# johannesulf/TabCorr

Measured on AMD Instinct MI355X. Metric: predict_calls_per_sec, higher is better.
Workload: dtype f64; 1 GPU; BASELINE configs[1]: Zheng07 predict(), synthetic auto table 50 mass bins x {cen,sat} (G=100, P=5050), 19 rp bins, n_gauss_prim=10, batch of 10000 draws per GPU per step, draws and results resident in HBM; n_tables=1, gather=none, gather_payload=ngal + xi (160 B per draw), gather_every_steps=32, lanes=4, rccl_ranks=0

## Files before the change

### include/tabcorr_amd_testing.h

```cpp
#ifndef TABCORR_AMD_TESTING_H
#define TABCORR_AMD_TESTING_H

#include "tabcorr_amd.h"

#ifdef __cplusplus
extern "C" {
#endif

int tc_debug_fastmath(int kind, int64_t n, const double* x, double* y);

int tc_debug_central_series(int n_gauss, double log_min, double log_max, double dist_index,
                            int64_t n, const double* log_m_min, const double* sigma,
                            double* series, double* nodes, int32_t* terms);

int tc_debug_satellite_series(int n_gauss, double log_min, double log_max, double dist_index,
                              int64_t n, const double* log_m0, const double* log_m1,
                              const double* alpha, double* series, double* nodes,
                              int32_t* terms);

int tc_plan_debug(int mode, int n_bins, const uint8_t* is_central, int n_chunks,
                  int64_t* n_entries, int32_t* entry_pair, int32_t* entry_chunk,
                  int32_t* entry_class);

int tc_debug_quad_schedule(int n_bins, int n_central, int by_type, int n_tiles, int n_rtiles,
                           int n_tables, int separate, int max_waves, int min_units,
                           int order ,
                           int* n_waves, int* n_runs, int* n_slabs, int64_t* units_min,
                           int64_t* units_max);
int tc_debug_triangle_parts(int n_rb, int n_parts, int32_t* rb0, int32_t* cb0, int32_t* count);
int tc_debug_node_groups(int n_bins, int n_central, const double* log_min,
                         const double* log_max, int32_t* begin, int32_t* member,
                         int* n_groups, int* n_central_groups);
int tc_debug_quad_emulate(int n_bins, int n_r, const double* tpcf_matrix,
                          const uint8_t* is_central, int by_type, int separate,
                          const double* densities, int64_t ldb, int64_t n_draws,
                          int max_waves, int min_units, int order, double* out);

int tc_debug_trace(tc_table* table, uint64_t* out, int64_t capacity, int64_t* n_blocks);
int tc_debug_wave_trace(tc_table* table, uint64_t* out, int64_t capacity,
                        int64_t* n_waves);
int tc_debug_resident_ticks(tc_table* table, uint64_t* out, int64_t capacity, int64_t* n_blocks);
int tc_debug_ensemble_stamps(tc_table* table, uint64_t* out);
#ifdef __cplusplus
}
// ... 4 lines not shown
```

### tabcorr_amd/_lib.py

```python

import ctypes
import os

import numpy as np

HERE = os.path.dirname(os.path.abspath(__file__))
LIBRARY = os.path.join(HERE, 'libtabcorr_hip.so')

TC_OK = 0
TC_ERR_INVALID = 1
TC_ERR_HIP = 2
TC_ERR_UNSUPPORTED = 3
TC_ERR_RCCL = 4

MODE = {'auto': 0, 'cross': 1}
DTYPE_F64 = 0
DTYPE_F32 = 1

FLAG_SEPARATE_GAL_TYPE = 1
FLAG_MODULATE_WITH_CENOCC = 2
FLAG_ASSEMBIAS = 4
FLAG_LEAUTHAUD11 = 16

UNIQUE_ID_BYTES = 128
# ... 18 lines not shown
    'tc_memcpy_h2d': [ctypes.c_void_p, ctypes.c_void_p, ctypes.c_size_t],
    'tc_memcpy_d2h': [ctypes.c_void_p, ctypes.c_void_p, ctypes.c_size_t],
    'tc_host_alloc': [c_void_pp, ctypes.c_size_t],
    'tc_host_free': [ctypes.c_void_p],
    'tc_host_register': [ctypes.c_void_p, ctypes.c_size_t],
    'tc_host_unregister': [ctypes.c_void_p],
    'tc_host_is_pinned': [ctypes.c_void_p, ctypes.c_size_t, c_int_p],
    'tc_gauss_legendre': [ctypes.c_int, c_double_p, c_double_p],
    'tc_debug_fastmath': [ctypes.c_int, ctypes.c_int64, c_double_p,
                          c_double_p],
    'tc_pair_indices': [ctypes.c_int, c_int32_p, c_int32_p, c_int32_p],
    'tc_spline_interpolation_matrix': [ctypes.c_int, c_double_p, c_double_p],
    'tc_plan_debug': [ctypes.c_int, ctypes.c_int, c_uint8_p, ctypes.c_int,
                      c_int64_p, c_int32_p, c_int32_p, c_int32_p],
    'tc_debug_triangle_parts': [ctypes.c_int, ctypes.c_int, c_int_p, c_int_p, c_int_p],
    'tc_debug_central_series': [ctypes.c_int, ctypes.c_double, ctypes.c_double, ctypes.c_double,
                                ctypes.c_int64, c_double_p, c_double_p, c_double_p, c_double_p,
                                c_int32_p],
    'tc_debug_satellite_series': [ctypes.c_int, ctypes.c_double, ctypes.c_double,
                                  ctypes.c_double, ctypes.c_int64, c_double_p, c_double_p,
                                  c_double_p, c_double_p, c_double_p, c_int32_p],
    'tc_debug_node_groups': [ctypes.c_int, ctypes.c_int, c_double_p, c_double_p,
                             c_int32_p, c_int32_p, c_int_p, c_int_p],
    'tc_debug_quad_schedule': [ctypes.c_int] * 10 + [c_int_p, c_int_p, c_int_p,
                                                     c_int64_p, c_int64_p],
    'tc_debug_quad_emulate': [ctypes.c_int, ctypes.c_int, c_double_p, c_uint8_p,
                              ctypes.c_int, ctypes.c_int, c_double_p,
                              ctypes.c_int64, ctypes.c_int64, ctypes.c_int,
                              ctypes.c_int, ctypes.c_int, c_double_p],
    'tc_table_create': [
# ... 210 lines not shown
```

### tabcorr_amd/csrc/hostmath.cpp

```cpp
#include "hostmath.h"
#include "fastmath.h"
#include "series.h"

#include <algorithm>
#include <atomic>
#include <cmath>
#include <cstring>
#include <map>
#include <numeric>
#include <tuple>
#include <thread>

namespace tc {

void gauss_legendre(int n, std::vector<double>& x, std::vector<double>& w) {
  x.assign(n, 0.0);
  w.assign(n, 0.0);
  const long double pi = 3.141592653589793238462643383279502884L;
  for (int i = 0; i < (n + 1) / 2; ++i) {
    long double z = cosl(pi * (i + 0.75L) / (n + 0.5L));
    long double dp = 1.0L;
    for (int iter = 0; iter < 100; ++iter) {
      long double p0 = 1.0L, p1 = z;
      for (int k = 2; k <= n; ++k) {
// ... 704 lines not shown
}

void triangle_parts(int n_rb, int n_parts, int32_t* rb0, int32_t* cb0, int32_t* count) {
  const int64_t n_units = (int64_t)n_rb * (n_rb + 1) / 2;
  for (int part = 0; part < n_parts; ++part) {
    const int64_t begin = n_units * part / n_parts, end = n_units * (part + 1) / n_parts;
    int64_t rb = (int64_t)((std::sqrt(8.0 * (double)begin + 1.0) - 1.0) / 2.0);
    while ((rb + 1) * (rb + 2) / 2 <= begin) ++rb;
    while (rb * (rb + 1) / 2 > begin) --rb;
    rb0[part] = (int32_t)rb;
    cb0[part] = (int32_t)(begin - rb * (rb + 1) / 2);
    count[part] = (int32_t)(end - begin);
  }
}

QuadTiling quad_tiling(int n_r) {
  QuadTiling tiling;
  tiling.n_rtiles = (n_r + 19) / 20;
  tiling.r_per_tile = (n_r + tiling.n_rtiles - 1) / tiling.n_rtiles;
  tiling.n_u = (tiling.r_per_tile + 3) / 4;
  return tiling;
}

void fill_quad_table(const QuadLayout& layout, const std::vector<int32_t>& perm, int n_r,
                     int64_t n_pairs, const void* matrix, bool matrix_is_f32,
                     const QuadTiling& tiling, std::vector<double>& out) {
  const int up = (tiling.n_u + 1) / 2;
  const size_t per_unit = (size_t)up * 128;
  out.assign((size_t)tiling.n_rtiles * layout.n_units * per_unit, 0.0);
  auto source = [&](int r, int64_t column) {
// ... 478 lines not shown
```

### tabcorr_amd/csrc/hostmath.h

```cpp
#pragma once

#include <cstdint>
#include <string>
#include <vector>

namespace tc {

void gauss_legendre(int n, std::vector<double>& x, std::vector<double>& w);

inline int64_t packed_index(int64_t i, int64_t j) {
  return i >= j ? i * (i + 1) / 2 + j : j * (j + 1) / 2 + i;
}

bool spline_interpolation_matrix(int n, const double* xp, std::vector<double>& a);

struct Segment {
  int32_t component;
  int32_t rectangular;
  int32_t i_lo, i_hi;
  int32_t j_lo, j_hi;
  int64_t q_begin;
  int64_t n_real;
};

// ... 114 lines not shown
  int32_t pad;
};
struct QuadMergePlan {
  int waves_per_block = 0;
  int n_blocks = 0;
  int lds_slots = 0;
  std::vector<int32_t> block_begin;
  std::vector<QuadMerge> merges;
};
void merge_quad_schedule(const QuadLayout& layout, int n_rtiles, bool separate,
                         int waves_per_block, int max_slots, QuadSchedule& schedule,
                         QuadMergePlan& plan);

void triangle_parts(int n_rb, int n_parts, int32_t* rb0, int32_t* cb0, int32_t* count);

struct QuadTiling {
  int n_rtiles = 1;
  int r_per_tile = 0;
  int n_u = 0;
};
QuadTiling quad_tiling(int n_r);

void fill_quad_table(const QuadLayout& layout, const std::vector<int32_t>& perm, int n_r,
                     int64_t n_pairs, const void* matrix, bool matrix_is_f32,
                     const QuadTiling& tiling, std::vector<double>& out);

QuadTiling quad_tiling_f32(int n_r);
void fill_quad_table_f32(const QuadLayout& layout, const std::vector<int32_t>& perm, int n_r,
                         int64_t n_pairs, const void* matrix, bool matrix_is_f32,
                         const QuadTiling& tiling, std::vector<float>& out);
// ... 47 lines not shown
```

### tabcorr_amd/csrc/internal.h

```cpp
#pragma once

#include <hip/hip_runtime.h>
#include <hip/hip_ext.h>

#include <algorithm>
#include <chrono>
#include <cmath>
#include <cstdarg>
#include <cstdio>
#include <cstdlib>
#include <cstring>
#include <map>
#include <memory>
#include <string>
#include <utility>
#include <vector>

#include "../../include/tabcorr_amd.h"
#include "../../include/tabcorr_amd_testing.h"
#include "fastmath.h"
#include "hostmath.h"
#include "kernel_args.h"

namespace tc {
// ... 217 lines not shown
  int occ_splits = 0;
  int occ_per_cu = 4;
  int n_groups = 0, n_waves = 0, lds_min = 0, min_chunk_entries = 32;
  int k_splits = 0;
  int trace = 0;
  int autotune_after = 0;
  int sync_chunks = 0;
  int sync_form = 32;
  int sync_stagger = 10;
  int sync_direct_out = 2;
  int async_direct_in = 1;
  int async_direct_out = 2;
  int series = -1;
  int cross_defer = 1;
  int fused_defer = 2;
  int fused_sat_cap = 6;
  int cross_wide_min_draws = 4096;
  int cross_target = 160;
  int resident_aperture = 1;
  int cross_min_draws = 192;
  int fused = 1;
  int fused_min_draws = 0;
  int fused_max_draws = 30720;
  int fused_waves = 0;
  int fused_draws = 0;
  int fused_spread = 1, fused_spread_min = 8192, fused_spread_rounds = 1;
  int prio_fused = 1, prio_fused_occ = 2, prio_fused_out = 3;
  int deterministic = 0;
  int skip_occ = 0, skip_finalize = 0;
  void load() {
// ... 63 lines not shown
  int n_r = 0;
  int64_t n_pairs = 0;
  int compute_dtype = TC_DTYPE_F64;
  bool legacy = false;
  tc::Plan plan;
  int rt = 0;
  int n_rtiles = 0;
  hipStream_t stream = nullptr;
  hipEvent_t ev_begin = nullptr, ev_end = nullptr;

  std::vector<double> n_h, log_min, log_max, percentile, dist_index;

  void* d_table = nullptr;
  size_t table_bytes = 0;
  void* d_n_h = nullptr;
  void* d_percentile = nullptr;
  void* d_perm = nullptr;
  tc::NodeGroups node_groups;
  void* d_group_begin = nullptr;
  void* d_group_member = nullptr;
  void* d_group_n_h = nullptr;
  void* d_group_percentile = nullptr;
  bool grouped = false;
  void* d_math_table = nullptr;
  void* d_pos_ij = nullptr;
  void* d_pos_off = nullptr;
  std::vector<double> cross_host;
  tc::host::CrossFused cross_fused, cross_fused_wide;
  int sync_cross_target = 0;
  std::vector<hipEvent_t> chunk_events;
// ... 225 lines not shown
```

### tabcorr_amd/csrc/kernel_args.h

```cpp
#pragma once

#include <cstdint>

#include "hostmath.h"

namespace tc {

constexpr int kLanes = 64;
constexpr unsigned kFlagSeparate = 1u;
constexpr unsigned kFlagModulate = 2u;
constexpr unsigned kFlagAssembias = 4u;
constexpr int kOccWaves = 4;
constexpr int kF32Block = 8;
constexpr int kF64Block = 8;
constexpr int kF32Tile = 32;
constexpr int kFinalizeRows = 32;
constexpr int kMaxInterpDim = 8;
constexpr int kMaxInterpAxis = 32;

struct GroupArgs {
  const int32_t* begin;
  const int32_t* member;
  const double* log_m;
  const double* m;
// ... 218 lines not shown
struct FusedArgs {
  const double* theta;
  int n_theta;
  int n_bins;
  int n_central;
  int n_gauss;
  int dens_rows;
  int part_rb0[kFusedMaxParts];
  int part_cb0[kFusedMaxParts];
  int part_count[kFusedMaxParts];
  int part_triangular[kFusedMaxParts];
  int part_n_cb[kFusedMaxParts];
  int part_i_row0[kFusedMaxParts];
  int part_j_row0[kFusedMaxParts];
  int part_unit_base[kFusedMaxParts];
  int separate;
  int n_r;
  int priority;
  int64_t n_draws;
  const double* log_m;
  const double* m;
  const double* weight;
  const double* n_h;
  const double* percentile;
  double split;
  const double* math_table;
  const void* table;
  uint32_t table_bytes;
  double* ngal;
  double* xi;
// ... 114 lines not shown
```

### tabcorr_amd/csrc/kernels.hip.h

```cpp
#pragma once

#include <hip/hip_runtime.h>

#include <cstdint>
#include <utility>

#include "fastmath.h"
#include "hostmath.h"
#include "kernel_args.h"
#include "series.h"

#ifdef TC_DEVELOPER_KNOBS
#define TC_TRACE(pointer) ((pointer) != nullptr)
#else
#define TC_TRACE(pointer) false
#endif

namespace tc {

static_assert(sizeof(QuadRun) == 32 && sizeof(QuadCompArgs) == 32, "read as 8 x int32");

typedef const __attribute__((address_space(4))) double* sc_f64;
typedef const __attribute__((address_space(4))) float* sc_f32;
typedef const __attribute__((address_space(4))) int32_t* sc_i32;
// ... 1892 lines not shown
      mma(t1, b1, false);
      __builtin_amdgcn_sched_barrier(0);
    } else {
      t0 = t1;
      b0 = b1;
    }
#pragma unroll
    for (int u = 0; u < UU; ++u)
#pragma unroll
      for (int v = 0; v < 4; ++v) {
        F[u][0] = fma(D[u][0][v], e[v].x, F[u][0]);
        F[u][1] = fma(D[u][1][v], e[v].y, F[u][1]);
      }
    ++rb;
    cb = 0;
  }
}

__device__ __forceinline__ int wave_prefix_sum(int value) {
  auto shifted = [](int x, auto control, auto rows) {
    return __builtin_amdgcn_update_dpp(0, x, decltype(control)::value, decltype(rows)::value, 0xf,
                                       false);
  };
  typedef std::integral_constant<int, 0xf> all_rows;
  value += shifted(value, std::integral_constant<int, 0x111>(), all_rows());
  value += shifted(value, std::integral_constant<int, 0x112>(), all_rows());
  value += shifted(value, std::integral_constant<int, 0x114>(), all_rows());
  value += shifted(value, std::integral_constant<int, 0x118>(), all_rows());
  value += shifted(value, std::integral_constant<int, 0x142>(), std::integral_constant<int, 0xa>());
  value += shifted(value, std::integral_constant<int, 0x143>(), std::integral_constant<int, 0xc>());
// ... 138 lines not shown
      stamps[blockIdx.x * 32 + which] = __builtin_amdgcn_s_memrealtime();
  };
  if (skip & 1)
    for (int idx = threadIdx.x; idx < a.n_bins * DL; idx += blockDim.x) fused_lds[idx] = 1e-3;
#else
  constexpr int skip = 0;
  const int n_bins_occ = a.n_bins;
  auto stamp = [](int) {};
  auto wave_stamp = [](int) {};
#endif
  stamp(0);
  set_priority((a.priority >> 2) & 3);
  const int lane = threadIdx.x & 63;
  const int wave = __builtin_amdgcn_readfirstlane(threadIdx.x >> 6);
  const int n_gauss = NGAUSS > 0 ? NGAUSS : a.n_gauss;
  {
    typedef double __attribute__((ext_vector_type(2))) double2v;
    const int hi = fm::kTableDoubles / 2;
    const double2v* src = (const double2v*)a.math_table;
    double2v* dst = (double2v*)table;
    for (int i = threadIdx.x; i < hi; i += blockDim.x) dst[i] = src[i];
  }
  for (int idx = a.n_bins * DL + threadIdx.x; idx < a.dens_rows * DL; idx += blockDim.x)
    dens[idx] = 0.0;
  __syncthreads();
  stamp(1);

  const int draw = DL != 32 ? lane : (lane & 31);
  const int half = DL != 32 ? 0 : (lane >> 5);
  const bool live = DL != 40 || lane < 40;
  auto dens_at = [&](int row, int d) -> double& {
    return dens[DL == 40 ? dens40(row, d) : row * DL + d];
  };
  const int64_t col = (int64_t)blockIdx.x * DL;
  const int64_t b0 = col + draw;
  const int64_t b = b0 < a.n_draws ? b0 : a.n_draws - 1;
  double norm;
  {
    const double* th = a.theta + b * a.n_theta;
    LeauthaudDraw ld;
    if (LEAUTHAUD) ld = prepare_leauthaud(table, kc, th);
    DrawParams dp = LEAUTHAUD ? prepare_draw(table, kc, 12.0, 1.0, 12.0, 13.0, 1.0, 0.0, 0.0)
                              : draw_params<ASSEMBIAS>(table, kc, th);
    series_setup<MODULATE>(dp, (GROUPED ? a.group.series : a.series) != nullptr && DL != 32,
                           (GROUPED ? a.group.sat_series : a.sat_series) != nullptr && DL != 32);
    sc_f64 log_m = (sc_f64)a.log_m;
    sc_f64 mass = (sc_f64)a.m;
    sc_f64 weight = (sc_f64)a.weight;
    sc_f64 weight_sum = weight + a.n_bins * n_gauss;
    sc_f64 n_h = (sc_f64)a.n_h;
    sc_f64 percentile = (sc_f64)a.percentile;
// ... 160 lines not shown
    stamp(3);
    red[0][wave][lane] = sum_cen;
    red[1][wave][lane] = sum_sat;
    __syncthreads();
    stamp(4);
    double n_cen = 0.0, n_sat = 0.0;
#pragma unroll
    for (int w = 0; w < W; ++w) {
      n_cen += red[0][w][lane];
      n_sat += red[1][w][lane];
    }
    const double total = (skip & 1) ? 1.0 : n_cen + n_sat;
    norm = total * total;
    if (wave == 0 && half == 0 && live && b0 < a.n_draws) {
      if (a.separate) {
        a.ngal[2 * b0] = n_cen;
        a.ngal[2 * b0 + 1] = n_sat;
      } else {
        a.ngal[b0] = total;
      }
    }
  }

  set_priority(a.priority & 3);
  const int c = lane & 15, kq = lane >> 4;
  double F[UP][2][2];
  constexpr int UA = DL == 40 ? (U > 3 ? 3 : U) : 1, UB = DL == 40 && U > 3 ? U - 3 : 1;
  double F40a[UA][10], F40b[UB][10];
  if (DL == 40) {
    const int part = wave;
    const unsigned off_a = ((lane & 0x30) | ((lane & 3) << 2) | ((lane >> 2) & 3)) * 16;
    const double* dens_b = dens + (a.part_j_row0[part] + (lane >> 4)) * 40 + (lane & 3) * 10;
    const double* dens_e = dens + (a.part_i_row0[part] + (lane >> 4)) * 40 + (lane & 3) * 10;
    const __amdgpu_buffer_rsrc_t rs_t =
// ... 23 lines not shown
    if (U > 3 && !(skip & 2))
      fused_quad_pass40<(U > 3 ? 3 : 0), UB>(rs_t, off_a, unit_bytes, dens_b, dens_e, rb, cb,
                                             count, triangular, n_cb, first_unit, F40b);
  } else {
    const int sub = wave / PARTS, part = wave % PARTS;
    const unsigned off_a = lane * 16;
    const double* dens_b =
        dens + (a.part_j_row0[part] + kq) * DL + sub * kQuadTile + 2 * c;
    const double* dens_e = dens + a.part_i_row0[part] * DL + sub * kQuadTile + 2 * c;
    const __amdgpu_buffer_rsrc_t rs_t =
        __builtin_amdgcn_make_buffer_rsrc((void*)a.table, 0, a.table_bytes, kBufferFlags);
    const int rb = a.part_rb0[part], cb = a.part_cb0[part], count = a.part_count[part];
    const bool triangular = a.part_triangular[part] != 0;
    const int n_cb = a.part_n_cb[part];
    const unsigned unit_base = (unsigned)a.part_unit_base[part];
#pragma unroll
    for (int p = 0; p < UP; ++p) {
      F[p][0][0] = F[p][0][1] = F[p][1][0] = F[p][1][1] = 0.0;
      if (skip & 2) continue;
      if (2 * p + 1 < U)
        fused_quad_pass<2, DL>(rs_t, off_a + p * 1024, UP * 1024, dens_b, dens_e, rb, cb, count,
                               triangular, n_cb, unit_base, F[p]);
      else
        fused_quad_pass<1, DL>(rs_t, off_a + p * 1024, UP * 1024, dens_b, dens_e, rb, cb, count,
                               triangular, n_cb, unit_base, F[p]);
    }
  }
  stamp(5);
  __syncthreads();
  stamp(8);
  if (DL == 40) {
    const int q = lane >> 4;
    auto share = [&](int sub, int g) {
      return sub < UA ? F40a[sub < UA ? sub : 0][g] : F40b[sub >= UA ? sub - UA : 0][g];
    };
    double* out = dens + (wave * (4 * U) + ((lane >> 2) & 3)) * 40 + (lane & 3);
    if (((a.priority >> 11) & 1) && __builtin_amdgcn_ballot_w64(!(norm < 1e280)) == 0) {
      double select[4];
#pragma unroll
      for (int m = 0; m < 4; ++m) select[m] = (lane & 3) == m ? 1.0 : 0.0;
#pragma unroll
      for (int sub = 0; sub < U; ++sub)
#pragma unroll
        for (int t = 0; t < 3; ++t) {
          double sums = 0.0;
// ... 77 lines not shown
    const int rows = a.n_r;
    const double* data = chi2_lds;
    const double* matrix = chi2_lds + rows;
    double part = 0.0;
    for (int i = wave; i < rows; i += W) {
      double inner = 0.0;
      for (int j = 0; j < rows; ++j)
        inner = fma(matrix[i * rows + j], tile[j][lane] - data[j], inner);
      part = fma(tile[i][lane] - data[i], inner, part);
    }
    red[0][wave][lane] = part;
    __syncthreads();
    if (wave == 0 && lane < n_valid) {
      double total = 0.0;
      for (int w = 0; w < W; ++w) total += red[0][w][lane];
      a.chi2[col + lane] = total;
    }
    return;
  }
  for (int idx = threadIdx.x; idx < a.n_r * DL; idx += blockDim.x) {
    const int d = idx / a.n_r, rr = idx % a.n_r;
    if (d < n_valid) a.xi[(col + d) * (int64_t)a.n_r + rr] = tile[rr][d];
  }
  stamp(7);
}

template <int ROW_LANES, typename Coefficient>
__device__ __forceinline__ void cross_deferred_pairs(
    const CrossFusedArgs& a, const double* table, const fm::Consts& kc, const DrawParams& dp,
    const unsigned long long* bitmap, unsigned* list, int wave, int lane, int g_first, int g_last,
    int type, Coefficient&& coefficient, double* res) {
  constexpr int SHARES = 64 / ROW_LANES;
  constexpr int SLOTS = 8 / SHARES;
  const int row = lane % ROW_LANES, share = lane / ROW_LANES;
  const unsigned long long owner = 0x0101010101010101ull << wave;
  double extra[SLOTS];
#pragma unroll
// ... 1787 lines not shown
```

### tabcorr_amd/csrc/launch.hip

```cpp
#include <immintrin.h>

#include <atomic>
#include <mutex>

#include "internal.h"
#include "kernels.hip.h"
#include "series.h"

namespace tc {
namespace host {

int get_quadrature(tc_table* t, int n_gauss, Quadrature** out) {
  auto it = t->quadrature.find(n_gauss);
  if (it != t->quadrature.end()) {
    *out = &it->second;
    return TC_OK;
  }
  std::vector<double> x, w;
  tc::gauss_legendre(n_gauss, x, w);
  const int g = t->n_bins;
  std::vector<double> log_m((size_t)g * n_gauss), m((size_t)g * n_gauss),
      weight((size_t)g * n_gauss + g);
  for (int i = 0; i < g; ++i) {
    const double d_log = t->log_max[i] - t->log_min[i];
// ... 916 lines not shown
  fa.n_theta = n_theta;
  fa.n_bins = t->n_bins;
  fa.n_central = t->plan.n_central;
  fa.n_gauss = n_gauss;
  fa.dens_rows = fused_dens_rows(t, separate);
  fa.separate = separate ? 1 : 0;
  const bool spread = fused_spread_eligible(t, n_draws, n_gauss, flags);
  const bool wide = !spread && fused_wide_tables(t, separate, n_gauss, flags);
  const bool half_tiles = !spread && !wide && fused_half_tiles(t, separate, n_draws, n_gauss, flags);
  const int waves = spread || wide || half_tiles ? 8 : fused_waves(t, separate, flags);
  const int draws = spread ? 40 : wide || half_tiles ? 32 : 64;
  const int n_parts = spread ? 8 : waves * 32 / draws;
  if (!separate) {
    const tc::QuadComp& comp = q_table.layout.comps[0];
    tc::triangle_parts(comp.n_rb, n_parts, fa.part_rb0, fa.part_cb0, fa.part_count);
    for (int part = 0; part < n_parts; ++part) {
      fa.part_triangular[part] = 1;
      fa.part_n_cb[part] = comp.n_cb;
      fa.part_i_row0[part] = comp.i_bin0;
      fa.part_j_row0[part] = comp.j_bin0;
      fa.part_unit_base[part] = (int)comp.unit_base;
    }
  } else {
    const int quarter = n_parts / 4;
    for (int part = 0; part < n_parts; ++part) {
      const int c = part < quarter ? 0 : part < 3 * quarter ? 1 : 2;
      const int first = c == 0 ? 0 : c == 1 ? quarter : 3 * quarter;
      const int pieces = c == 1 ? 2 * quarter : quarter, piece = part - first;
      const tc::QuadComp& comp = q_table.layout.comps[c];
      fa.part_triangular[part] = comp.triangular;
// ... 9 lines not shown
        fa.part_count[part] = count[piece];
      } else {
        const int64_t begin = comp.n_units * piece / pieces;
        const int64_t end = comp.n_units * (piece + 1) / pieces;
        fa.part_rb0[part] = (int)(begin / comp.n_cb);
        fa.part_cb0[part] = (int)(begin % comp.n_cb);
        fa.part_count[part] = (int)(end - begin);
      }
    }
  }
  fa.n_r = t->n_r;
  fa.priority = (t->tuning.prio_fused & 3) | ((t->tuning.prio_fused_occ & 3) << 2) |
                ((t->tuning.prio_fused_out & 3) << 4) |
                ((env_int_early("TC_FUSED_SKIP", 0) & 3) << 8) |
                (q_table.finite ? 1 << 11 : 0);
  fa.n_draws = n_draws;
  fa.n_groups = t->node_groups.n_groups;
  fa.n_central_groups = t->node_groups.n_central_groups;
  fa.group = group_args(t, *q);
  fa.series = (series_mask(t) & 1) ? (const double*)q->series : nullptr;
  fa.series_thr = (const int32_t*)q->series_thr;
  fa.sat_series = (series_mask(t) & 2) ? (const double*)q->sat_series : nullptr;
  fa.sat_series_thr = (const int32_t*)q->sat_series_thr;
  fa.log_m = (const double*)q->log_m;
  fa.m = (const double*)q->m;
  fa.weight = (const double*)q->weight;
  fa.n_h = (const double*)t->d_n_h;
  fa.percentile = (const double*)t->d_percentile;
  fa.split = 0.5;
  fa.math_table = (const double*)t->d_math_table;
// ... 994 lines not shown
```

### tabcorr_amd/csrc/runtime.cpp

```cpp
#include <dlfcn.h>
#include <pthread.h>

#include <atomic>
#include <condition_variable>
#include <mutex>
#include <new>
#include <thread>
#include <vector>

#include "internal.h"
#include "series.h"

namespace tc {
namespace host {

namespace {
thread_local std::string g_last_error;
}

namespace {
struct Roctx {
  int (*push)(const char*) = nullptr;
  int (*pop)() = nullptr;
};
// ... 631 lines not shown
        entry_chunk[e] = c;
        entry_class[e] = chunk.component;
        ++e;
      }
    }
  }
  for (int64_t q = 0; q < plan.n_positions; ++q)
    if (!seen[q]) return fail(TC_ERR_INVALID, "position %lld not covered", (long long)q);
  if (e != plan.n_entries) return fail(TC_ERR_INVALID, "entries missing");
  return TC_OK;
}

int tc_debug_triangle_parts(int n_rb, int n_parts, int32_t* rb0, int32_t* cb0, int32_t* count) {
  TC_CHECK(n_rb >= 1 && n_parts >= 1 && rb0 && cb0 && count, "invalid argument");
  tc::triangle_parts(n_rb, n_parts, rb0, cb0, count);
  return TC_OK;
}

int tc_debug_quad_schedule(int n_bins, int n_central, int by_type, int n_tiles, int n_rtiles,
                           int n_tables, int separate, int max_waves, int min_units, int order,
                           int* n_waves, int* n_runs, int* n_slabs, int64_t* units_min,
                           int64_t* units_max) {
  TC_CHECK(n_bins >= 1 && n_central >= 0 && n_central <= n_bins && n_tiles >= 1 &&
               n_rtiles >= 1 && max_waves >= 1,
           "invalid arguments");
  tc::QuadLayout layout;
  tc::build_quad_layout(n_bins, n_central, by_type != 0, layout);
  tc::QuadSchedule schedule;
  tc::build_quad_schedule(layout, n_tiles, n_rtiles, n_tables, separate != 0, max_waves,
                          min_units, schedule, order);
// ... 91 lines not shown
```

### tabcorr_amd/csrc/table.cpp

```cpp
#include <cmath>

#include "internal.h"

using namespace tc::host;

extern "C" {

int tc_table_create(int mode, int n_bins, int n_r, int64_t n_pairs,
                    const void* tpcf_matrix, int matrix_dtype, const double* n_h,
                    const double* log_min, const double* log_max,
                    const double* percentile, const double* dist_index,
                    const uint8_t* is_central, int compute_dtype, tc_table** out) {
  TC_CHECK(out != nullptr, "table output pointer is NULL");
  *out = nullptr;
  TC_CHECK(mode == TC_MODE_AUTO || mode == TC_MODE_CROSS, "invalid mode %d", mode);
  TC_CHECK(n_bins >= 1 && n_bins < (1 << 20), "invalid number of bins %d", n_bins);
  TC_CHECK(n_r >= 1, "invalid number of correlation function bins %d", n_r);
  const int64_t expect =
      mode == TC_MODE_AUTO ? (int64_t)n_bins * (n_bins + 1) / 2 : n_bins;
  TC_CHECK(n_pairs == expect,
           "tpcf_matrix has %lld columns but %d bins in mode '%s' need %lld",
           (long long)n_pairs, n_bins, mode == TC_MODE_AUTO ? "auto" : "cross",
           (long long)expect);
  TC_CHECK(n_pairs < (1LL << 31), "too many pair columns");
// ... 113 lines not shown
    for (int l = 0; l < t->n_lanes; ++l) t->lanes[l].stream = streams[l];
    if (created != TC_OK) return created;
    for (int l = 0; l < t->n_lanes; ++l)
      TC_HIP(hipEventCreateWithFlags(&t->lanes[l].finished, hipEventDisableTiming));
  }
  t->stream = t->lanes[0].stream;
  TC_HIP(hipEventCreate(&t->ev_begin));
  TC_HIP(hipEventCreate(&t->ev_end));
  int status = compute_dtype == TC_DTYPE_F64 ? upload(tmp64, &t->d_table)
                                             : upload(tmp32, &t->d_table);
  if (status == TC_OK && compute_dtype == TC_DTYPE_F32)
    status = upload(pos_ij, &t->d_pos_ij);
  if (status == TC_OK && compute_dtype == TC_DTYPE_F64)
    status = upload(pos_ij, &t->d_pos_off);
  if (status == TC_OK) status = upload(t->n_h, &t->d_n_h);
  if (status == TC_OK) status = upload(t->percentile, &t->d_percentile);
  if (status == TC_OK) status = upload(t->plan.perm, &t->d_perm);
  tc::find_node_groups(n_bins, t->plan.n_central, t->log_min.data(), t->log_max.data(),
                       t->node_groups);
  t->grouped = t->node_groups.largest > 1;
  if (status == TC_OK) status = upload(t->node_groups.begin, &t->d_group_begin);
  if (status == TC_OK) status = upload(t->node_groups.member, &t->d_group_member);
  {
    std::vector<double> n_h_m, percentile_m;
    for (int32_t g : t->node_groups.member) {
      n_h_m.push_back(t->n_h[g]);
      percentile_m.push_back(t->percentile[g]);
    }
    if (status == TC_OK) status = upload(n_h_m, &t->d_group_n_h);
    if (status == TC_OK) status = upload(percentile_m, &t->d_group_percentile);
// ... 26 lines not shown

int tc_table_destroy(tc_table* t) {
  if (t == nullptr) return TC_OK;
  (void)hipSetDevice(t->device);
  (void)resident_stop(t);
  if (t->resident.stream) (void)hipStreamDestroy(t->resident.stream);
  t->resident.mailbox.release();
  t->resident.ens_mailbox.release();
  t->resident.ens_out.release();
  t->resident.ens_device.release();
  t->resident.ens_aperture.release();
  t->resident.single_aperture.release();
  t->resident.ws.buffer.release();
  for (tc_table::Lane& lane : t->lanes)
    if (lane.stream) (void)hipStreamSynchronize(lane.stream);
  for (void* p : {t->d_table, t->d_n_h, t->d_percentile, t->d_perm, t->d_math_table,
                  t->d_pos_ij, t->d_pos_off, t->d_group_begin, t->d_group_member,
                  t->d_group_n_h, t->d_group_percentile})
    if (p) (void)hipFree(p);
  for (auto& kv : t->quadrature)
    for (void* p : {kv.second.log_m, kv.second.m, kv.second.weight, kv.second.group_log_m,
                    kv.second.group_m, kv.second.group_weight, kv.second.series,
                    kv.second.series_thr, kv.second.group_series, kv.second.group_series_thr,
                    kv.second.sat_series, kv.second.sat_series_thr, kv.second.group_sat_series,
                    kv.second.group_sat_series_thr, kv.second.group_records, kv.second.sat_records, kv.second.cen_records})
      if (p) (void)hipFree(p);
  for (auto& kv : t->chunkings)
    for (void* p : {kv.second->chunks, kv.second->groups})
      if (p) (void)hipFree(p);
  t->quad_by_type.release();
  t->quad_total.release();
// ... 1073 lines not shown
  } else if (key == "resident_aperture") {
    TC_CHECK(value == 0 || value == 1, "resident_aperture must be 0 or 1");
    const int status = resident_stop(t);
    if (status != TC_OK) return status;
    t->tuning.resident_aperture = value;
    t->resident.ens_grid = 0;
    t->resident.single_aperture_decided = false;
  } else if (key == "cross_min_draws") {
    TC_CHECK(value >= 1, "cross_min_draws must be positive");
    t->tuning.cross_min_draws = value;
  } else if (key == "cross_defer") {
    t->tuning.cross_defer = value != 0;
  } else if (key == "fused_defer") {
    TC_CHECK(value >= 0 && value <= 2, "fused_defer must be 0, 1 or 2");
    t->tuning.fused_defer = value;
  } else if (key == "fused_sat_cap") {
    TC_CHECK(value >= 0 && value <= 6, "fused_sat_cap must be in [0, 6]");
    t->tuning.fused_sat_cap = value;
  } else if (key == "cross_wide_min_draws") {
    TC_CHECK(value >= 0, "cross_wide_min_draws must not be negative");
    t->tuning.cross_wide_min_draws = value;
  } else if (key == "cross_target") {
    TC_CHECK(value >= 1 && value <= 4096, "cross_target must be in [1, 4096]");
    t->tuning.cross_target = value;
  } else if (key == "series") {
    TC_CHECK(value >= -1 && value <= 3, "series must be -1 .. 3");
    t->tuning.series = value;
  } else if (key == "grouped") {
    t->grouped = value != 0 && t->node_groups.largest > 1;
  } else if (key == "lanes") {
// ... 215 lines not shown
```

Before: 271.9 million calls/s.

## Skip empty density blocks in fused quad and sort draws by satellite cutoff

Adds a row-set based quadrature pass for the non-separate fused kernel that ballots which 4-bin density blocks are nonzero across the wave and skips MFMA work on dead blocks. To make those blocks dead for whole waves, each block ranks draws by how many satellite block upper mass limits their log_M0 exceeds, using an in-LDS counting sort, and processes draws in that sorted order, scattering ngal, xi and chi2 back to the original indices. Rows are assigned to parts by greedy balancing instead of contiguous triangle ranges. The cost is a per-block histogram/rank prologue over all draws and more irregular control flow in the MFMA loop.

```diff
diff --git a/include/tabcorr_amd_testing.h b/include/tabcorr_amd_testing.h
--- a/include/tabcorr_amd_testing.h
+++ b/include/tabcorr_amd_testing.h
@@ -28,6 +28,8 @@
                            int* n_waves, int* n_runs, int* n_slabs, int64_t* units_min,
                            int64_t* units_max);
 int tc_debug_triangle_parts(int n_rb, int n_parts, int32_t* rb0, int32_t* cb0, int32_t* count);
+
+int tc_debug_triangle_row_parts(int n_rb, int n_parts, uint64_t* rows);
 int tc_debug_node_groups(int n_bins, int n_central, const double* log_min,
                          const double* log_max, int32_t* begin, int32_t* member,
                          int* n_groups, int* n_central_groups);
diff --git a/tabcorr_amd/_lib.py b/tabcorr_amd/_lib.py
--- a/tabcorr_amd/_lib.py
+++ b/tabcorr_amd/_lib.py
@@ -56,6 +56,8 @@
     'tc_plan_debug': [ctypes.c_int, ctypes.c_int, c_uint8_p, ctypes.c_int,
                       c_int64_p, c_int32_p, c_int32_p, c_int32_p],
     'tc_debug_triangle_parts': [ctypes.c_int, ctypes.c_int, c_int_p, c_int_p, c_int_p],
+    'tc_debug_triangle_row_parts': [ctypes.c_int, ctypes.c_int,
+                                    ctypes.POINTER(ctypes.c_uint64)],
     'tc_debug_central_series': [ctypes.c_int, ctypes.c_double, ctypes.c_double, ctypes.c_double,
                                 ctypes.c_int64, c_double_p, c_double_p, c_double_p, c_double_p,
                                 c_int32_p],
diff --git a/tabcorr_amd/csrc/hostmath.cpp b/tabcorr_amd/csrc/hostmath.cpp
--- a/tabcorr_amd/csrc/hostmath.cpp
+++ b/tabcorr_amd/csrc/hostmath.cpp
@@ -742,6 +742,31 @@
   }
 }
 
+void triangle_row_parts(int n_rb, int n_parts, uint64_t* rows) {
+  std::vector<int64_t> units(n_parts, 0);
+  for (int part = 0; part < n_parts; ++part) rows[part] = 0;
+  int above = -1;
+  for (int rb = n_rb - 1; rb >= 0; --rb) {
+    int best = -1;
+    for (int part = 0; part < n_parts; ++part)
+      if ((part != above || n_parts == 1) && (best < 0 || units[part] < units[best])) best = part;
+    units[best] += rb + 1;
+    rows[best] |= (uint64_t)1 << rb;
+    above = best;
+  }
+}
+
+void satellite_block_tops(int n_bins, int n_central, const double* log_max,
+                          std::vector<double>& tops) {
+  tops.clear();
+  for (int first = (n_central + 3) / 4 * 4; first < n_bins; first += 4) {
+    double top = log_max[first];
+    for (int g = first; g < n_bins && g < first + 4; ++g) top = std::max(top, log_max[g]);
+    if (top == top) tops.push_back(top);
+  }
+  std::sort(tops.begin(), tops.end());
+}
+
 QuadTiling quad_tiling(int n_r) {
   QuadTiling tiling;
   tiling.n_rtiles = (n_r + 19) / 20;
diff --git a/tabcorr_amd/csrc/hostmath.h b/tabcorr_amd/csrc/hostmath.h
--- a/tabcorr_amd/csrc/hostmath.h
+++ b/tabcorr_amd/csrc/hostmath.h
@@ -152,6 +152,11 @@
 
 void triangle_parts(int n_rb, int n_parts, int32_t* rb0, int32_t* cb0, int32_t* count);
 
+void triangle_row_parts(int n_rb, int n_parts, uint64_t* rows);
+
+void satellite_block_tops(int n_bins, int n_central, const double* log_max,
+                          std::vector<double>& tops);
+
 struct QuadTiling {
   int n_rtiles = 1;
   int r_per_tile = 0;
diff --git a/tabcorr_amd/csrc/internal.h b/tabcorr_amd/csrc/internal.h
--- a/tabcorr_amd/csrc/internal.h
+++ b/tabcorr_amd/csrc/internal.h
@@ -255,6 +255,7 @@
   int series = -1;
   int cross_defer = 1;
   int fused_defer = 2;
+  int fused_skip = 1;
   int fused_sat_cap = 6;
   int cross_wide_min_draws = 4096;
   int cross_target = 160;
@@ -348,6 +349,8 @@
   void* d_table = nullptr;
   size_t table_bytes = 0;
   void* d_n_h = nullptr;
+  std::vector<double> block_tops;
+  void* d_block_tops = nullptr;
   void* d_percentile = nullptr;
   void* d_perm = nullptr;
   tc::NodeGroups node_groups;
diff --git a/tabcorr_amd/csrc/kernel_args.h b/tabcorr_amd/csrc/kernel_args.h
--- a/tabcorr_amd/csrc/kernel_args.h
+++ b/tabcorr_amd/csrc/kernel_args.h
@@ -256,6 +256,9 @@
   int part_i_row0[kFusedMaxParts];
   int part_j_row0[kFusedMaxParts];
   int part_unit_base[kFusedMaxParts];
+  unsigned long long part_rows[kFusedMaxParts];
+  const double* block_tops;
+  int n_block_tops;
   int separate;
   int n_r;
   int priority;
diff --git a/tabcorr_amd/csrc/kernels.hip.h b/tabcorr_amd/csrc/kernels.hip.h
--- a/tabcorr_amd/csrc/kernels.hip.h
+++ b/tabcorr_amd/csrc/kernels.hip.h
@@ -1930,6 +1930,117 @@
       }
     ++rb;
     cb = 0;
+  }
+}
+
+template <int UU, int DL>
+__device__ __forceinline__ void fused_quad_rows(__amdgpu_buffer_rsrc_t rs_t, unsigned off_a,
+                                                unsigned unit_bytes, const double* dens_b,
+                                                const double* dens_e, unsigned long long rows,
+                                                unsigned long long live, unsigned unit_base,
+                                                double (&F)[2][2]) {
+  rows &= live;
+  if (rows == 0) return;
+  f64x2 t0, t1, b0, b1, e[4];
+  f64x4 D[UU][2];
+  auto mma = [&](const f64x2& t, const f64x2& b, bool first) {
+    if (first) {
+      const f64x4 zero = {0.0, 0.0, 0.0, 0.0};
+#pragma unroll
+      for (int u = 0; u < UU; ++u) {
+        const double av = u ? t.y : t.x;
+        D[u][0] = __builtin_amdgcn_mfma_f64_16x16x4f64(av, b.x, zero, 0, 0, 0);
+        D[u][1] = __builtin_amdgcn_mfma_f64_16x16x4f64(av, b.y, zero, 0, 0, 0);
+      }
+    } else {
+#pragma unroll
+      for (int u = 0; u < UU; ++u) {
+        const double av = u ? t.y : t.x;
+        D[u][0] = __builtin_amdgcn_mfma_f64_16x16x4f64(av, b.x, D[u][0], 0, 0, 0);
+        D[u][1] = __builtin_amdgcn_mfma_f64_16x16x4f64(av, b.y, D[u][1], 0, 0, 0);
+      }
+    }
+  };
+  auto first_run = [&](unsigned long long& columns, int& column, int& length) {
+    column = __builtin_ctzll(columns);
+    length = __builtin_ctzll(~(columns >> column));
+    columns &= ~0ull << (column + length);
+  };
+  auto unit_offset = [&](int row, int column) {
+    return (unit_base + (unsigned)(row * (row + 1) / 2 + column)) * unit_bytes;
+  };
+  int rb = __builtin_ctzll(rows);
+  rows &= rows - 1;
+  unsigned long long cols = live & ((2ull << rb) - 1);
+  int cb, n;
+  first_run(cols, cb, n);
+  unsigned ua = unit_offset(rb, cb);
+  bool row_begins = true;
+  t0 = buffer_load16<0>(rs_t, off_a, ua);
+  b0 = *(const f64x2*)(dens_b + 4 * cb * DL);
+  ua += unit_bytes;
+  for (;;) {
+    const bool row_ends = cols == 0;
+    const bool more = !row_ends || rows != 0;
+    int next_rb = rb, next_cb = cb, next_n = 0;
+    unsigned long long next_cols = cols;
+    if (row_ends && rows != 0) {
+      next_rb = __builtin_ctzll(rows);
+      rows &= rows - 1;
+      next_cols = live & ((2ull << next_rb) - 1);
+    }
+    if (more) first_run(next_cols, next_cb, next_n);
+    const unsigned next_ua = unit_offset(next_rb, next_cb);
+    auto fetch = [&](f64x2& t, f64x2& b, int k) {
+      const bool inside = k < n;
+      t = buffer_load16<0>(rs_t, off_a, inside ? ua : next_ua);
+      b = *(const f64x2*)(dens_b + 4 * (inside ? cb + k : next_cb) * DL);
+      ua += unit_bytes;
+    };
+    if (row_begins) {
+#pragma unroll
+      for (int v = 0; v < 4; ++v) e[v] = *(const f64x2*)(dens_e + (4 * rb + v) * DL);
+    }
+    fetch(t1, b1, 1);
+    __builtin_amdgcn_sched_barrier(0);
+    if (row_begins) mma(t0, b0, true); else mma(t0, b0, false);
+    __builtin_amdgcn_sched_barrier(0);
+    int t = 1;
+    for (; t + 1 < n; t += 2) {
+      fetch(t0, b0, t + 1);
+      __builtin_amdgcn_sched_barrier(0);
+      mma(t1, b1, false);
+      __builtin_amdgcn_sched_barrier(0);
+      fetch(t1, b1, t + 2);
+      __builtin_amdgcn_sched_barrier(0);
+      mma(t0, b0, false);
+      __builtin_amdgcn_sched_barrier(0);
+    }
+    if (t < n) {
+      fetch(t0, b0, n);
+      __builtin_amdgcn_sched_barrier(0);
+      mma(t1, b1, false);
+      __builtin_amdgcn_sched_barrier(0);
+    } else {
+      t0 = t1;
+      b0 = b1;
+    }
+    if (row_ends) {
+#pragma unroll
+      for (int u = 0; u < UU; ++u)
+#pragma unroll
+        for (int v = 0; v < 4; ++v) {
+          F[u][0] = fma(D[u][0][v], e[v].x, F[u][0]);
+          F[u][1] = fma(D[u][1][v], e[v].y, F[u][1]);
+        }
+    }
+    if (!more) break;
+    rb = next_rb;
+    cb = next_cb;
+    n = next_n;
+    cols = next_cols;
+    row_begins = row_ends;
+    ua = next_ua + unit_bytes;
   }
 }
 
@@ -2098,6 +2209,97 @@
   const int lane = threadIdx.x & 63;
   const int wave = __builtin_amdgcn_readfirstlane(threadIdx.x >> 6);
   const int n_gauss = NGAUSS > 0 ? NGAUSS : a.n_gauss;
+  constexpr bool kCanRank = DL == 64 && W == 8 && !LEAUTHAUD;
+  const bool ranked = kCanRank && ((a.priority >> 14) & 1);
+  int64_t ranked_draw = 0;
+  if (kCanRank && ranked) {
+    const int n = (int)a.n_draws;
+    const int n_keys = a.n_block_tops + 1;
+    const int n_chunks = (n + 63) >> 6, chunk_stride = (n_chunks + 3) & ~3;
+    unsigned char* keys = (unsigned char*)fused_lds;
+    unsigned* counts = (unsigned*)(keys + ((n + 15) & ~15));
+    unsigned* hist = (unsigned*)(table + fm::kTableDoubles);
+    unsigned* key_begin = hist + 64;
+    unsigned* wave_count = key_begin + 68;
+    int* order = (int*)(wave_count + W * 64);
+    for (int idx = threadIdx.x; idx < n_keys * chunk_stride / 4; idx += blockDim.x) counts[idx] = 0;
+    if (threadIdx.x < 64) hist[threadIdx.x] = 0;
+    __syncthreads();
+    sc_f64 tops = (sc_f64)a.block_tops;
+    for (int base = 0; base < n; base += 4 * 64 * W) {
+      double log_m0[4];
+      int key[4];
+#pragma unroll
+      for (int u = 0; u < 4; ++u) {
+        const int i = base + u * 64 * W + (int)threadIdx.x;
+        log_m0[u] = a.theta[(int64_t)(i < n ? i : n - 1) * a.n_theta + 2];
+        key[u] = 0;
+      }
+      for (int k = 0; k < a.n_block_tops; ++k) {
+        const double top = tops[k];
+#pragma unroll
+        for (int u = 0; u < 4; ++u) key[u] += log_m0[u] >= top ? 1 : 0;
+      }
+#pragma unroll
+      for (int u = 0; u < 4; ++u) {
+        const int i = base + u * 64 * W + (int)threadIdx.x;
+        if (i < n) {
+          keys[i] = (unsigned char)key[u];
+          atomicAdd(&hist[key[u]], 1u);
+          const int at = key[u] * chunk_stride + (i >> 6);
+          atomicAdd(&counts[at >> 2], 1u << (8 * (at & 3)));
+        }
+      }
+    }
+    __syncthreads();
+    if (wave == 0) {
+      const int inclusive = wave_prefix_sum(lane < n_keys ? (int)hist[lane] : 0);
+      key_begin[lane + 1] = (unsigned)inclusive;
+      if (lane == 0) key_begin[0] = 0;
+    }
+    __syncthreads();
+    const int64_t wanted = (int64_t)blockIdx.x * 64 + lane;
+    const unsigned rank = (unsigned)(wanted < n ? wanted : n - 1);
+    int key = 0;
+    for (int k = 1; k < n_keys; ++k) key += key_begin[k] <= rank ? 1 : 0;
+    const unsigned place = rank - key_begin[key];
+    const unsigned char* of_key = (const unsigned char*)counts + key * chunk_stride;
+    const int per_wave = (n_chunks + W - 1) / W;
+    {
+      unsigned sum = 0;
+      const int end = (wave + 1) * per_wave < n_chunks ? (wave + 1) * per_wave : n_chunks;
+      for (int c = wave * per_wave; c < end; ++c) sum += of_key[c];
+      wave_count[wave * 64 + lane] = sum;
+    }
+    __syncthreads();
+    if (wave == 0) {
+      unsigned before = 0;
+      int w = 0;
+      for (; w < W - 1; ++w) {
+        const unsigned here = wave_count[w * 64 + lane];
+        if (before + here > place) break;
+        before += here;
+      }
+      int c = w * per_wave;
+      for (; c < n_chunks - 1; ++c) {
+        const unsigned here = of_key[c];
+        if (before + here > place) break;
+        before += here;
+      }
+      int found = c * 64;
+      for (int j = 0; j < 64 && c * 64 + j < n; ++j) {
+        if (keys[c * 64 + j] == (unsigned char)key) {
+          found = c * 64 + j;
+          if (before == place) break;
+          ++before;
+        }
+      }
+      order[lane] = found < n ? found : n - 1;
+    }
+    __syncthreads();
+    ranked_draw = order[lane];
+    __syncthreads();
+  }
   {
     typedef double __attribute__((ext_vector_type(2))) double2v;
     const int hi = fm::kTableDoubles / 2;
@@ -2118,7 +2320,7 @@
   };
   const int64_t col = (int64_t)blockIdx.x * DL;
   const int64_t b0 = col + draw;
-  const int64_t b = b0 < a.n_draws ? b0 : a.n_draws - 1;
+  const int64_t b = kCanRank && ranked ? ranked_draw : b0 < a.n_draws ? b0 : a.n_draws - 1;
   double norm;
   {
     const double* th = a.theta + b * a.n_theta;
@@ -2309,10 +2511,10 @@
     norm = total * total;
     if (wave == 0 && half == 0 && live && b0 < a.n_draws) {
       if (a.separate) {
-        a.ngal[2 * b0] = n_cen;
-        a.ngal[2 * b0 + 1] = n_sat;
+        a.ngal[2 * b] = n_cen;
+        a.ngal[2 * b + 1] = n_sat;
       } else {
-        a.ngal[b0] = total;
+        a.ngal[b] = total;
       }
     }
   }
@@ -2366,10 +2568,33 @@
     const bool triangular = a.part_triangular[part] != 0;
     const int n_cb = a.part_n_cb[part];
     const unsigned unit_base = (unsigned)a.part_unit_base[part];
+    unsigned long long live_blocks = ~0ull;
+    if (!a.separate && ((a.priority >> 13) & 1) && ((a.priority >> 11) & 1)) {
+      unsigned long long unsafe = __builtin_amdgcn_ballot_w64(!(norm < 1e280));
+      unsafe &= DL == 32 ? 0xffffffffull : sub ? 0xffffffff00000000ull : 0xffffffffull;
+      if (unsafe == 0) {
+        const double* mine = dens + 2 * (lane >> 5) * DL + sub * kQuadTile + (lane & 31);
+        live_blocks = 0;
+        const int n_blocks = a.dens_rows >> 2;
+        for (int k = 0; k < n_blocks; ++k) {
+          const bool occupied = mine[4 * k * DL] != 0.0 || mine[(4 * k + 1) * DL] != 0.0;
+          if (__builtin_amdgcn_ballot_w64(occupied) != 0) live_blocks |= 1ull << k;
+        }
+      }
+    }
 #pragma unroll
     for (int p = 0; p < UP; ++p) {
       F[p][0][0] = F[p][0][1] = F[p][1][0] = F[p][1][1] = 0.0;
       if (skip & 2) continue;
+      if (!a.separate) {
+        if (2 * p + 1 < U)
+          fused_quad_rows<2, DL>(rs_t, off_a + p * 1024, UP * 1024, dens_b, dens_e,
+                                 a.part_rows[part], live_blocks, unit_base, F[p]);
+        else
+          fused_quad_rows<1, DL>(rs_t, off_a + p * 1024, UP * 1024, dens_b, dens_e,
+                                 a.part_rows[part], live_blocks, unit_base, F[p]);
+        continue;
+      }
       if (2 * p + 1 < U)
         fused_quad_pass<2, DL>(rs_t, off_a + p * 1024, UP * 1024, dens_b, dens_e, rb, cb, count,
                                triangular, n_cb, unit_base, F[p]);
@@ -2381,6 +2606,8 @@
   stamp(5);
   __syncthreads();
   stamp(8);
+  long long* const draw_index = (long long*)&red[1][0][0];
+  if (kCanRank && ranked && wave == 0) draw_index[lane] = b;
   if (DL == 40) {
     const int q = lane >> 4;
     auto share = [&](int sub, int g) {
@@ -2488,13 +2715,15 @@
     if (wave == 0 && lane < n_valid) {
       double total = 0.0;
       for (int w = 0; w < W; ++w) total += red[0][w][lane];
-      a.chi2[col + lane] = total;
+      a.chi2[kCanRank && ranked ? b : col + lane] = total;
     }
     return;
   }
   for (int idx = threadIdx.x; idx < a.n_r * DL; idx += blockDim.x) {
     const int d = idx / a.n_r, rr = idx % a.n_r;
-    if (d < n_valid) a.xi[(col + d) * (int64_t)a.n_r + rr] = tile[rr][d];
+    if (d < n_valid)
+      a.xi[(kCanRank && ranked ? (int64_t)draw_index[d] : col + d) * (int64_t)a.n_r + rr] =
+          tile[rr][d];
   }
   stamp(7);
 }
diff --git a/tabcorr_amd/csrc/launch.hip b/tabcorr_amd/csrc/launch.hip
--- a/tabcorr_amd/csrc/launch.hip
+++ b/tabcorr_amd/csrc/launch.hip
@@ -954,6 +954,12 @@
   if (!separate) {
     const tc::QuadComp& comp = q_table.layout.comps[0];
     tc::triangle_parts(comp.n_rb, n_parts, fa.part_rb0, fa.part_cb0, fa.part_count);
+    if (!spread) {
+      if (comp.n_rb > 62) return fail(TC_ERR_INVALID, "more than 62 block rows");
+      uint64_t rows[tc::kFusedMaxParts];
+      tc::triangle_row_parts(comp.n_rb, n_parts, rows);
+      for (int part = 0; part < n_parts; ++part) fa.part_rows[part] = rows[part];
+    }
     for (int part = 0; part < n_parts; ++part) {
       fa.part_triangular[part] = 1;
       fa.part_n_cb[part] = comp.n_cb;
@@ -993,6 +999,22 @@
                 ((t->tuning.prio_fused_out & 3) << 4) |
                 ((env_int_early("TC_FUSED_SKIP", 0) & 3) << 8) |
                 (q_table.finite ? 1 << 11 : 0);
+  if (t->tuning.fused_skip != 0 && !separate && !spread &&
+      q_table.layout.comps[0].i_bin0 == 0 && q_table.layout.comps[0].j_bin0 == 0) {
+    fa.priority |= 1 << 13;
+    const int64_t n_keys = (int64_t)t->block_tops.size() + 1;
+    const int64_t chunks = ((n_draws + 63) / 64 + 3) / 4 * 4;
+    const int64_t rank_bytes = (n_draws + 15) / 16 * 16 + n_keys * chunks;
+    const int64_t room =
+        (int64_t)std::max(fa.dens_rows * draws, tc::fused_slot_doubles(waves, draws)) * 8;
+    if (draws == 64 && waves == 8 && !(flags & TC_FLAG_LEAUTHAUD11) && n_theta >= 3 &&
+        t->d_block_tops != nullptr && n_keys <= 63 && n_draws > 64 && n_draws <= 32768 &&
+        rank_bytes <= room) {
+      fa.priority |= 1 << 14;
+      fa.block_tops = (const double*)t->d_block_tops;
+      fa.n_block_tops = (int)t->block_tops.size();
+    }
+  }
   fa.n_draws = n_draws;
   fa.n_groups = t->node_groups.n_groups;
   fa.n_central_groups = t->node_groups.n_central_groups;
diff --git a/tabcorr_amd/csrc/runtime.cpp b/tabcorr_amd/csrc/runtime.cpp
--- a/tabcorr_amd/csrc/runtime.cpp
+++ b/tabcorr_amd/csrc/runtime.cpp
@@ -669,6 +669,12 @@
 int tc_debug_triangle_parts(int n_rb, int n_parts, int32_t* rb0, int32_t* cb0, int32_t* count) {
   TC_CHECK(n_rb >= 1 && n_parts >= 1 && rb0 && cb0 && count, "invalid argument");
   tc::triangle_parts(n_rb, n_parts, rb0, cb0, count);
+  return TC_OK;
+}
+
+int tc_debug_triangle_row_parts(int n_rb, int n_parts, uint64_t* rows) {
+  TC_CHECK(n_rb >= 1 && n_rb <= 64 && n_parts >= 1 && rows, "invalid argument");
+  tc::triangle_row_parts(n_rb, n_parts, rows);
   return TC_OK;
 }
 
diff --git a/tabcorr_amd/csrc/table.cpp b/tabcorr_amd/csrc/table.cpp
--- a/tabcorr_amd/csrc/table.cpp
+++ b/tabcorr_amd/csrc/table.cpp
@@ -151,6 +151,9 @@
   if (status == TC_OK && compute_dtype == TC_DTYPE_F64)
     status = upload(pos_ij, &t->d_pos_off);
   if (status == TC_OK) status = upload(t->n_h, &t->d_n_h);
+  tc::satellite_block_tops(n_bins, t->plan.n_central, t->log_max.data(), t->block_tops);
+  if (status == TC_OK && !t->block_tops.empty())
+    status = upload(t->block_tops, &t->d_block_tops);
   if (status == TC_OK) status = upload(t->percentile, &t->d_percentile);
   if (status == TC_OK) status = upload(t->plan.perm, &t->d_perm);
   tc::find_node_groups(n_bins, t->plan.n_central, t->log_min.data(), t->log_max.data(),
@@ -207,7 +210,7 @@
   t->resident.ws.buffer.release();
   for (tc_table::Lane& lane : t->lanes)
     if (lane.stream) (void)hipStreamSynchronize(lane.stream);
-  for (void* p : {t->d_table, t->d_n_h, t->d_percentile, t->d_perm, t->d_math_table,
+  for (void* p : {t->d_table, t->d_n_h, t->d_block_tops, t->d_percentile, t->d_perm, t->d_math_table,
                   t->d_pos_ij, t->d_pos_off, t->d_group_begin, t->d_group_member,
                   t->d_group_n_h, t->d_group_percentile})
     if (p) (void)hipFree(p);
@@ -1311,6 +1314,9 @@
   } else if (key == "fused_defer") {
     TC_CHECK(value >= 0 && value <= 2, "fused_defer must be 0, 1 or 2");
     t->tuning.fused_defer = value;
+  } else if (key == "fused_skip") {
+    TC_CHECK(value == 0 || value == 1, "fused_skip must be 0 or 1");
+    t->tuning.fused_skip = value;
   } else if (key == "fused_sat_cap") {
     TC_CHECK(value >= 0 && value <= 6, "fused_sat_cap must be in [0, 6]");
     t->tuning.fused_sat_cap = value;
```

After: 263.8 million calls/s. 3.0% lower.
